# matter-labs/era-zkevm_test_harness

Measured on AMD Instinct MI355X. Metric: base-layer circuits/sec (2^20 rows); full-block synth wall-time 1/8 GPU, higher is better.
Workload: dtype u64 (Goldilocks, p = 2^64 - 2^32 + 1)

## Files before the change

### era_zkevm_test_harness_amd/csrc/poseidon2.cuh

```cuda
#pragma once
#include "gl64.cuh"
#include "../../include/zkw_poseidon2_params.h"

namespace p2 {
using gl::u32;
using gl::u64;

static __constant__ u64 c_rc[P2_TOTAL_ROUNDS * P2_WIDTH] = P2_ROUND_CONSTANTS_INIT;
static __constant__ u32 c_shift[P2_WIDTH] = P2_INTERNAL_DIAG_SHIFTS_INIT;

__host__ __device__ __forceinline__ u64 rc_at(int i) {
#if defined(__HIP_DEVICE_COMPILE__)
    return c_rc[i];
#else
    return P2_ROUND_CONSTANTS[i];
#endif
}
__host__ __device__ __forceinline__ u32 shift_at(int i) {
#if defined(__HIP_DEVICE_COMPILE__)
    return c_shift[i];
#else
    return P2_INTERNAL_DIAG_SHIFTS[i];
#endif
}

struct Wide {
    u64 lo;
    u32 hi;
};
GL_HD Wide wide(u64 x) { Wide r; r.lo = x; r.hi = 0; return r; }
GL_HD Wide wadd(Wide a, Wide b) {
    Wide r;
    r.lo = a.lo + b.lo;
    r.hi = a.hi + b.hi + (r.lo < a.lo ? 1u : 0u);
    return r;
}
GL_HD Wide wshl(Wide a, u32 s) {
    Wide r;
    r.lo = a.lo << s;
    r.hi = (a.hi << s) | (u32)(a.lo >> (64 - s));
    return r;
}
GL_HD u64 wreduce(Wide a) {
    u64 t = ((u64)a.hi << 32) - a.hi;
    u64 r = a.lo + t;
    u64 c = r < t ? gl::EPS : 0;
    return r + c;
}

GL_HD void m4w(const u64 x[4], Wide t[4]) {
    Wide t0 = wadd(wide(x[0]), wide(x[1])), t1 = wadd(wide(x[2]), wide(x[3]));
    Wide t2 = wadd(wshl(wide(x[1]), 1), t1), t3 = wadd(wshl(wide(x[3]), 1), t0);
    Wide t4 = wadd(wshl(t1, 2), t3), t5 = wadd(wshl(t0, 2), t2);
    t[0] = wadd(t3, t5); t[1] = t5; t[2] = wadd(t2, t4); t[3] = t4;
}

#if defined(__HIP_DEVICE_COMPILE__)
__device__ __forceinline__ u64 mad_acc(u32 a, u32 k, u64 acc) {
    u64 r, dead;
    asm("v_mad_u64_u32 %0, %1, %2, %3, %4" : "=v"(r), "=s"(dead) : "v"(a), "s"(k), "v"(acc));
    return r;
}
__device__ __forceinline__ u64 mad_acc1(u32 a, u64 acc) {
    u64 r, dead;
    asm("v_mad_u64_u32 %0, %1, %2, 1, %3" : "=v"(r), "=s"(dead) : "v"(a), "v"(acc));
    return r;
}
__device__ __forceinline__ u64 mad_acc2(u32 a, u64 acc) {
    u64 r, dead;
    asm("v_mad_u64_u32 %0, %1, %2, 2, %3" : "=v"(r), "=s"(dead) : "v"(a), "v"(acc));
    return r;
}
__device__ __forceinline__ u64 wp_reduce(u64 L, u64 H) {
    const u32 l0 = (u32)L, l1 = (u32)(L >> 32), h0 = (u32)H, h1 = (u32)(H >> 32);
    u32 n1, k, f;
    u64 c, c2, dead, r;
    asm("v_add_co_u32_e64 %0, %1, %2, %3" : "=v"(n1), "=s"(c) : "v"(l1), "v"(h0));
    asm("v_addc_co_u32_e64 %0, %1, %2, 0, %3" : "=v"(k), "=s"(dead) : "v"(h1), "s"(c));
    const u64 x = ((u64)n1 << 32) | l0;
    asm("v_mad_u64_u32 %0, %1, %2, -1, %3" : "=v"(r), "=s"(c2) : "v"(k), "v"(x));
    asm("v_cndmask_b32_e64 %0, 0, 1, %1" : "=v"(f) : "s"(c2));
    asm("v_mad_u64_u32 %0, %1, %2, -1, %3" : "=v"(r), "=s"(dead) : "v"(f), "v"(r));
    return r;
}
__device__ __forceinline__ void m4_plane(u32 a0, u32 a1, u32 a2, u32 a3, u64 y[4]) {
    const u64 t0 = mad_acc1(a0, (u64)a1), t1 = mad_acc1(a2, (u64)a3);
    const u64 t2 = mad_acc2(a1, t1), t3 = mad_acc2(a3, t0);
    const u64 t4 = (t1 << 2) + t3, t5 = (t0 << 2) + t2;
    y[0] = t3 + t5; y[1] = t5; y[2] = t2 + t4; y[3] = t4;
}
#endif

GL_HD void external(u64 s[12]) {
#if defined(__HIP_DEVICE_COMPILE__) && !defined(P2_LINEAR_WIDE)
    u64 L[12], H[12];
#pragma unroll
    for (int b = 0; b < 3; b++) {
        m4_plane((u32)s[4 * b], (u32)s[4 * b + 1], (u32)s[4 * b + 2], (u32)s[4 * b + 3], L + 4 * b);
        m4_plane((u32)(s[4 * b] >> 32), (u32)(s[4 * b + 1] >> 32), (u32)(s[4 * b + 2] >> 32), (u32)(s[4 * b + 3] >> 32), H + 4 * b);
    }
#pragma unroll
    for (int i = 0; i < 4; i++) {
        const u64 cl = L[i] + L[4 + i] + L[8 + i], ch = H[i] + H[4 + i] + H[8 + i];
#pragma unroll
        for (int b = 0; b < 3; b++) s[4 * b + i] = wp_reduce(L[4 * b + i] + cl, H[4 * b + i] + ch);
    }
#else
    Wide t[12];
    m4w(s, t); m4w(s + 4, t + 4); m4w(s + 8, t + 8);
#pragma unroll
    for (int i = 0; i < 4; i++) {
        Wide col = wadd(wadd(t[i], t[4 + i]), t[8 + i]);
        s[i] = wreduce(wadd(t[i], col)); s[4 + i] = wreduce(wadd(t[4 + i], col)); s[8 + i] = wreduce(wadd(t[8 + i], col));
    }
#endif
}

GL_HD void internal(u64 s[12]) {
    constexpr u32 SH[12] = P2_INTERNAL_DIAG_SHIFTS_INIT;
#if defined(__HIP_DEVICE_COMPILE__) && !defined(P2_LINEAR_WIDE)
    u64 sl = (u64)(u32)s[0], sh = s[0] >> 32;
#pragma unroll
    for (int i = 1; i < 12; i++) { sl = mad_acc1((u32)s[i], sl); sh = mad_acc1((u32)(s[i] >> 32), sh); }
#pragma unroll
    for (int i = 0; i < 12; i++) {
        const u64 l = SH[i] ? mad_acc((u32)s[i], 1u << SH[i], sl) : mad_acc1((u32)s[i], sl);
        const u64 h = SH[i] ? mad_acc((u32)(s[i] >> 32), 1u << SH[i], sh) : mad_acc1((u32)(s[i] >> 32), sh);
        s[i] = wp_reduce(l, h);
    }
#else
    Wide sum = wide(s[0]);
#pragma unroll
    for (int i = 1; i < 12; i++) sum = wadd(sum, wide(s[i]));
#pragma unroll
    for (int i = 0; i < 12; i++) s[i] = wreduce(wadd(SH[i] ? wshl(wide(s[i]), SH[i]) : wide(s[i]), sum));
#endif
}

#ifndef P2_SBOX_GROUP
#define P2_SBOX_GROUP 3
#endif
template <bool LAT = false>
GL_HD void full_round(u64 s[12], int r) {
#pragma unroll
    for (int i = 0; i < 12; i++) {
        s[i] = LAT ? gl::pow7_lat(gl::add_canon(s[i], rc_at(12 * r + i))) : gl::pow7(gl::add_canon(s[i], rc_at(12 * r + i)));
#if defined(__HIP_DEVICE_COMPILE__)
        if (!LAT && (i + 1) % P2_SBOX_GROUP == 0) __builtin_amdgcn_sched_barrier(0);
#endif
    }
    external(s);
}

template <bool LAT = false>
GL_HD void partial_round(u64 s[12], int r) {
    s[0] = LAT ? gl::pow7_lat(gl::add_canon(s[0], rc_at(12 * r))) : gl::pow7(gl::add_canon(s[0], rc_at(12 * r)));
    internal(s);
}

template <bool LAT = false>
GL_HD void permute(u64 s[12]) {
    external(s);
    int r = 0;
    for (int k = 0; k < P2_HALF_FULL_ROUNDS; k++, r++) full_round<LAT>(s, r);
    for (int k = 0; k < P2_PARTIAL_ROUNDS; k++, r++) partial_round<LAT>(s, r);
    for (int k = 0; k < P2_HALF_FULL_ROUNDS; k++, r++) full_round<LAT>(s, r);
}
GL_HD void permute_lat(u64 s[12]) { permute<true>(s); }

#if defined(__HIPCC__)
template <int CTRL>
__device__ __forceinline__ u32 dpp32(u32 v) {
    return (u32)__builtin_amdgcn_update_dpp((int)0, (int)v, CTRL, 0xF, 0xF, false);
}
template <int CTRL>
__device__ __forceinline__ u64 dpp64(u64 v) {
    u32 lo = dpp32<CTRL>((u32)v), hi = dpp32<CTRL>((u32)(v >> 32));
    return ((u64)hi << 32) | lo;
}
constexpr int QP_ROT1 = 1 | (2 << 2) | (3 << 4) | (0 << 6);
constexpr int QP_ROT2 = 2 | (3 << 2) | (0 << 4) | (1 << 6);
constexpr int QP_ROT3 = 3 | (0 << 2) | (1 << 4) | (2 << 6);
constexpr int QP_SWAP1 = 1 | (0 << 2) | (3 << 4) | (2 << 6);
constexpr int QP_BCAST0 = 0;
constexpr int ROW_ROR4 = 0x124, ROW_ROR8 = 0x128, ROW_ROR12 = 0x12C;

template <int CTRL>
__device__ __forceinline__ Wide wdpp(Wide a) {
    Wide r;
    r.lo = dpp64<CTRL>(a.lo);
    r.hi = dpp32<CTRL>(a.hi);
    return r;
}
__device__ __forceinline__ u64 add_rc_sched(u64 x, u64 c) {
    u32 r0, r1, m;
    asm("v_add_co_u32 %0, vcc, %3, %5\n\t"
        "v_addc_co_u32 %1, vcc, %4, %6, vcc\n\t"
        "v_cndmask_b32 %2, 0, -1, vcc\n\t"
        "v_add_co_u32 %0, vcc, %0, %2\n\t"
        "v_addc_co_u32 %1, vcc, 0, %1, vcc"
        : "=&v"(r0), "=&v"(r1), "=&v"(m)
        : "v"((u32)x), "v"((u32)(x >> 32)), "v"((u32)c), "v"((u32)(c >> 32))
        : "vcc");
    return ((u64)r1 << 32) | r0;
}
#if defined(GL_CHAIN_MUL_COMPILER_FORM)
#define P2_ROW_MUL gl::mul_sched
#else
#define P2_ROW_MUL gl::mul_vcc
#endif
__device__ __forceinline__ u64 pow7_sched(u64 x) {
    const u64 x2 = P2_ROW_MUL(x, x), x3 = P2_ROW_MUL(x2, x), x4 = P2_ROW_MUL(x2, x2);
    return P2_ROW_MUL(x3, x4);
}

struct Coop {
    u64 rc_full[2 * P2_HALF_FULL_ROUNDS];
    u32 ka, kb, kd;
    u32 shift;
    u32 rsh, hi_mask;
    bool active;
    bool first;
    bool second;

    __device__ __forceinline__ void init(int g) {
        active = g < 12;
        first = g == 0;
        second = g == 1;
#pragma unroll
        for (int k = 0; k < 2 * P2_HALF_FULL_ROUNDS; k++) {
            int round = k < P2_HALF_FULL_ROUNDS ? k : k + P2_PARTIAL_ROUNDS;
            rc_full[k] = active ? c_rc[12 * round + g] : 0;
        }
        bool even = (g & 1) == 0;
        ka = even ? 5u : 6u;
        kb = even ? 7u : 1u;
        kd = even ? 3u : 4u;
        shift = active ? c_shift[g] : 0;
        rsh = (32u - shift) & 31u;
        hi_mask = shift ? 0xffffffffu : 0u;
    }

    __device__ __forceinline__ u64 external(u64 x) const {
        u64 a = x, b = dpp64<QP_ROT1>(x), c = dpp64<QP_ROT2>(x), d = dpp64<QP_ROT3>(x);
        u64 L = (a & gl::EPS) * ka + (b & gl::EPS) * kb + (c & gl::EPS) + (d & gl::EPS) * kd;
        u64 H = (a >> 32) * ka + (b >> 32) * kb + (c >> 32) + (d >> 32) * kd;
        u32 r0, r1, t0, t1, t2, u0, u1, u2, e0, e1, e2;
        asm volatile(
            "v_add_co_u32 %3, vcc, %11, %13\n\t"
            "v_addc_co_u32 %4, vcc, 0, %14, vcc\n\t"
            "s_nop 0\n\t"
            "v_add_co_u32_dpp %5, vcc, %12, %12 row_ror:8 row_mask:0xf bank_mask:0xf\n\t"
            "v_addc_co_u32_dpp %6, vcc, %3, %3, vcc row_ror:8 row_mask:0xf bank_mask:0xf\n\t"
            "v_addc_co_u32_dpp %7, vcc, %4, %4, vcc row_ror:8 row_mask:0xf bank_mask:0xf\n\t"
            "v_add_co_u32_dpp %5, vcc, %5, %5 row_ror:4 row_mask:0xf bank_mask:0xf\n\t"
            "v_addc_co_u32_dpp %6, vcc, %6, %6, vcc row_ror:4 row_mask:0xf bank_mask:0xf\n\t"
            "v_addc_co_u32_dpp %7, vcc, %7, %7, vcc row_ror:4 row_mask:0xf bank_mask:0xf\n\t"
            "v_add_co_u32 %0, vcc, %12, %5\n\t"
            "v_addc_co_u32 %1, vcc, %3, %6, vcc\n\t"
            "v_addc_co_u32 %2, vcc, %4, %7, vcc\n\t"
            "v_sub_co_u32 %8, vcc, 0, %2\n\t"
            "v_subbrev_co_u32 %9, vcc, 0, %2, vcc\n\t"
            "v_add_co_u32 %0, vcc, %0, %8\n\t"
            "v_addc_co_u32 %1, vcc, %1, %9, vcc\n\t"
            "v_cndmask_b32 %10, 0, -1, vcc\n\t"
            "v_add_co_u32 %0, vcc, %0, %10\n\t"
            "v_addc_co_u32 %1, vcc, 0, %1, vcc"
            : "=&v"(r0), "=&v"(r1), "=&v"(t0), "=&v"(t1), "=&v"(t2), "=&v"(u0), "=&v"(u1), "=&v"(u2), "=&v"(e0), "=&v"(e1), "=&v"(e2)
            : "v"((u32)(L >> 32)), "v"((u32)L), "v"((u32)H), "v"((u32)(H >> 32))
            : "vcc");
        const u64 y = ((u64)r1 << 32) | r0;
        return active ? y : 0;
    }

    __device__ __forceinline__ u64 internal(u64 x) const {
        const u32 x0 = (u32)x, x1 = (u32)(x >> 32);
        u32 s0, s1, s2;
        const u32 zero = 0;
        asm volatile(
            "s_nop 1\n\t"
            "v_add_co_u32_dpp %0, vcc, %3, %3 row_ror:8 row_mask:0xf bank_mask:0xf\n\t"
            "v_addc_co_u32_dpp %1, vcc, %4, %4, vcc row_ror:8 row_mask:0xf bank_mask:0xf\n\t"
            "v_addc_co_u32 %2, vcc, 0, %5, vcc\n\t"
            "v_add_co_u32_dpp %0, vcc, %0, %0 row_ror:4 row_mask:0xf bank_mask:0xf\n\t"
            "v_addc_co_u32_dpp %1, vcc, %1, %1, vcc row_ror:4 row_mask:0xf bank_mask:0xf\n\t"
            "v_addc_co_u32_dpp %2, vcc, %2, %2, vcc row_ror:4 row_mask:0xf bank_mask:0xf\n\t"
            "v_add_co_u32_dpp %0, vcc, %0, %0 quad_perm:[2,3,0,1] row_mask:0xf bank_mask:0xf\n\t"
            "v_addc_co_u32_dpp %1, vcc, %1, %1, vcc quad_perm:[2,3,0,1] row_mask:0xf bank_mask:0xf\n\t"
            "v_addc_co_u32_dpp %2, vcc, %2, %2, vcc quad_perm:[2,3,0,1] row_mask:0xf bank_mask:0xf\n\t"
            "v_add_co_u32_dpp %0, vcc, %0, %0 quad_perm:[1,0,3,2] row_mask:0xf bank_mask:0xf\n\t"
            "v_addc_co_u32_dpp %1, vcc, %1, %1, vcc quad_perm:[1,0,3,2] row_mask:0xf bank_mask:0xf\n\t"
            "v_addc_co_u32_dpp %2, vcc, %2, %2, vcc quad_perm:[1,0,3,2] row_mask:0xf bank_mask:0xf"
            : "=&v"(s0), "=&v"(s1), "=&v"(s2)
            : "v"(x0), "v"(x1), "v"(zero)
            : "vcc");
        const u64 mlo = x << shift;
        const u32 m2 = (x1 >> rsh) & hi_mask;
        u32 r0, r1;
        u32 t0, t1, t2, t3;
        asm volatile(
            "v_add_co_u32 %0, vcc, %6, %9\n\t"
            "v_addc_co_u32 %1, vcc, %7, %10, vcc\n\t"
            "v_addc_co_u32 %2, vcc, %8, %11, vcc\n\t"
            "v_sub_co_u32 %3, vcc, 0, %2\n\t"
            "v_subbrev_co_u32 %4, vcc, 0, %2, vcc\n\t"
            "v_add_co_u32 %0, vcc, %0, %3\n\t"
            "v_addc_co_u32 %1, vcc, %1, %4, vcc\n\t"
            "v_cndmask_b32 %5, 0, -1, vcc\n\t"
            "v_add_co_u32 %0, vcc, %0, %5\n\t"
            "v_addc_co_u32 %1, vcc, 0, %1, vcc"
            : "=&v"(r0), "=&v"(r1), "=&v"(t0), "=&v"(t1), "=&v"(t2), "=&v"(t3)
            : "v"((u32)mlo), "v"((u32)(mlo >> 32)), "v"(m2), "v"(s0), "v"(s1), "v"(s2)
            : "vcc");
        const u64 y = ((u64)r1 << 32) | r0;
        return active ? y : 0;
    }

    __device__ __forceinline__ u64 permute(u64 x) const {
        x = external(x);
#pragma unroll
        for (int k = 0; k < P2_HALF_FULL_ROUNDS; k++) x = external(pow7_sched(add_rc_sched(x, rc_full[k])));
        for (int k = 0; k < P2_PARTIAL_ROUNDS; k++) {
            u64 rc = c_rc[12 * (P2_HALF_FULL_ROUNDS + k)];
            u64 sx = pow7_pair(add_rc_sched(x, rc));
            x = internal(first ? sx : x);
        }
#pragma unroll
        for (int k = 0; k < P2_HALF_FULL_ROUNDS; k++)
            x = external(pow7_sched(add_rc_sched(x, rc_full[P2_HALF_FULL_ROUNDS + k])));
        return x;
    }

    __device__ __forceinline__ u64 pow7_pair(u64 t) const {
        const u64 t0 = dpp64<QP_BCAST0>(t);
        const u64 x2 = P2_ROW_MUL(t0, t0);
        const u64 b = second ? x2 : t0;
        const u64 y = P2_ROW_MUL(x2, b);
        return P2_ROW_MUL(y, dpp64<QP_SWAP1>(y));
    }
};

template <class Put>
__device__ __forceinline__ u64 coop_flattened(const Coop& co, u64 x, u32 g, Put&& put) {
    if (co.active) put(g, gl::canon(x));
    x = co.external(x);
#pragma unroll
    for (int k = 0; k < P2_HALF_FULL_ROUNDS; k++) {
        x = co.external(pow7_sched(add_rc_sched(x, co.rc_full[k])));
        if (co.active) put(12 * (k + 1) + g, gl::canon(x));
    }
    for (int k = 0; k < P2_PARTIAL_ROUNDS; k++) {
        const u64 rc = c_rc[12 * (P2_HALF_FULL_ROUNDS + k)];
        const u64 sx = co.pow7_pair(add_rc_sched(x, rc));
        if (co.first) put(12 * (P2_HALF_FULL_ROUNDS + 1) + k, gl::canon(sx));
        x = co.internal(co.first ? sx : x);
    }
#pragma unroll
    for (int k = 0; k < P2_HALF_FULL_ROUNDS; k++) {
        x = co.external(pow7_sched(add_rc_sched(x, co.rc_full[P2_HALF_FULL_ROUNDS + k])));
        if (co.active) put(12 * (P2_HALF_FULL_ROUNDS + 1) + P2_PARTIAL_ROUNDS + 12 * k + g, gl::canon(x));
    }
    return gl::canon(x);
}


__device__ __forceinline__ u64 q4_mul(u64 a, u64 b) {
#if defined(GL_CHAIN_MUL_COMPILER_FORM)
    return gl::mul_lat(a, b);
#else
    return gl::mul_vcc(a, b);
#endif
}
__device__ __forceinline__ u64 q4_pow7(u64 x) {
    const u64 x2 = q4_mul(x, x), x3 = q4_mul(x2, x), x4 = q4_mul(x2, x2);
    return q4_mul(x3, x4);
}
template <int CTRL>
__device__ __forceinline__ u32 qdpp32(u32 v) {
    return (u32)__builtin_amdgcn_update_dpp((int)0, (int)v, CTRL, 0xF, 0xF, true);
}
template <int CTRL>
__device__ __forceinline__ u64 qdpp64(u64 v) {
    return ((u64)qdpp32<CTRL>((u32)(v >> 32)) << 32) | qdpp32<CTRL>((u32)v);
}

struct Coop4 {
    u64 rc_full[2 * P2_HALF_FULL_ROUNDS][3];
    u32 ka, kb, kd;
    u32 pw[3];
    bool first;
    bool second;

    __device__ __forceinline__ void init(int j) {
        first = j == 0;
        second = j == 1;
#pragma unroll
        for (int k = 0; k < 2 * P2_HALF_FULL_ROUNDS; k++) {
            int round = k < P2_HALF_FULL_ROUNDS ? k : k + P2_PARTIAL_ROUNDS;
#pragma unroll
            for (int c = 0; c < 3; c++) rc_full[k][c] = c_rc[12 * round + 4 * c + j];
        }
        bool even = (j & 1) == 0;
        ka = even ? 5u : 6u;
        kb = even ? 7u : 1u;
        kd = even ? 3u : 4u;
#pragma unroll
        for (int c = 0; c < 3; c++) pw[c] = 1u << c_shift[4 * c + j];
    }

#if defined(__HIP_DEVICE_COMPILE__)
    static __device__ __forceinline__ u64 mad_v(u32 a, u32 k, u64 acc) {
        u64 r, dead;
        asm("v_mad_u64_u32 %0, %1, %2, %3, %4" : "=v"(r), "=s"(dead) : "v"(a), "v"(k), "v"(acc));
        return r;
    }
    template <bool SC = false>
    static __device__ __forceinline__ u64 add_rc(u64 x, u32 c0, u32 c1);
#endif

    __device__ __forceinline__ u64 m4_plane(u32 a) const {
        const u32 b = qdpp32<QP_ROT1>(a), c = qdpp32<QP_ROT2>(a), d = qdpp32<QP_ROT3>(a);
#if defined(__HIP_DEVICE_COMPILE__)
        return mad_v(d, kd, mad_v(b, kb, mad_v(a, ka, (u64)c)));
#else
        return (u64)a * ka + (u64)b * kb + c + (u64)d * kd;
#endif
    }

    __device__ __forceinline__ void external(u64 x[3]) const {
#if defined(__HIP_DEVICE_COMPILE__)
        u64 L[3], H[3];
#pragma unroll
        for (int c = 0; c < 3; c++) { L[c] = m4_plane((u32)x[c]); H[c] = m4_plane((u32)(x[c] >> 32)); }
        const u64 cl = L[0] + L[1] + L[2], ch = H[0] + H[1] + H[2];
#pragma unroll
        for (int c = 0; c < 3; c++) x[c] = wp_reduce(L[c] + cl, H[c] + ch);
#endif
    }

    __device__ __forceinline__ void internal(u64 x[3]) const {
#if defined(__HIP_DEVICE_COMPILE__)
        const u64 pl = mad_acc1((u32)x[0], mad_acc1((u32)x[1], (u64)(u32)x[2]));
        const u64 ph = mad_acc1((u32)(x[0] >> 32), mad_acc1((u32)(x[1] >> 32), x[2] >> 32));
        u32 l0, l1, h0, h1;
        asm volatile(
            "s_nop 1\n\t"
            "v_add_co_u32_dpp %0, vcc, %4, %4 quad_perm:[2,3,0,1] row_mask:0xf bank_mask:0xf\n\t"
            "v_addc_co_u32_dpp %1, vcc, %5, %5, vcc quad_perm:[2,3,0,1] row_mask:0xf bank_mask:0xf\n\t"
            "v_add_co_u32_dpp %2, vcc, %6, %6 quad_perm:[2,3,0,1] row_mask:0xf bank_mask:0xf\n\t"
            "v_addc_co_u32_dpp %3, vcc, %7, %7, vcc quad_perm:[2,3,0,1] row_mask:0xf bank_mask:0xf\n\t"
            "v_add_co_u32_dpp %0, vcc, %0, %0 quad_perm:[1,0,3,2] row_mask:0xf bank_mask:0xf\n\t"
            "v_addc_co_u32_dpp %1, vcc, %1, %1, vcc quad_perm:[1,0,3,2] row_mask:0xf bank_mask:0xf\n\t"
            "v_add_co_u32_dpp %2, vcc, %2, %2 quad_perm:[1,0,3,2] row_mask:0xf bank_mask:0xf\n\t"
            "v_addc_co_u32_dpp %3, vcc, %3, %3, vcc quad_perm:[1,0,3,2] row_mask:0xf bank_mask:0xf"
            : "=&v"(l0), "=&v"(l1), "=&v"(h0), "=&v"(h1)
            : "v"((u32)pl), "v"((u32)(pl >> 32)), "v"((u32)ph), "v"((u32)(ph >> 32))
            : "vcc");
        const u64 sl = ((u64)l1 << 32) | l0, sh = ((u64)h1 << 32) | h0;
#pragma unroll
        for (int c = 0; c < 3; c++) x[c] = wp_reduce(mad_v((u32)x[c], pw[c], sl), mad_v((u32)(x[c] >> 32), pw[c], sh));
#endif
    }

    __device__ __forceinline__ void permute(u64 x[3]) const {
#if defined(__HIP_DEVICE_COMPILE__)
        constexpr u64 RC[P2_TOTAL_ROUNDS * P2_WIDTH] = P2_ROUND_CONSTANTS_INIT;
        external(x);
#pragma unroll
// ... 124 lines not shown
```

### era_zkevm_test_harness_amd/csrc/ram_circuit_kernels.cuh

```cuda
#pragma once
#include "../../include/zkw_ram_circuit_spec.h"
#include "../../include/zkw_decommit_sorter_circuit_spec.h"
#include "../../include/zkw_events_sorter_circuit_spec.h"
#include "ram_kernels.cuh"
#include "public_input_kernels.cuh"
#include "closed_form_kernels.cuh"

namespace zkw {

struct SynthJob {
    const zkw_ram_instance* inst;
    const zkw_mem_query* sorted_q;
    const zkw_mem_query* unsorted_q;
    const u64* unsorted_caps;
    const u64* sorted_caps;
    const u64* u_mark;
    const u64* s_mark;
    const u64* challenges;
    const u64* gp_ckpt;
    u64* trace;
    u32* hist;
    const u32* nd_tiles;
    const u64* public_input;
    const zkw_ram_instance* first_inst;
    u32 tail_clean;
};

constexpr int RC_INLINE_JOBS = 32;
struct SynthJobsRef {
    const SynthJob* p;
    __device__ __forceinline__ const SynthJob& operator[](unsigned k) const { return p[k]; }
};
struct SynthJobsInline {
    SynthJob j[RC_INLINE_JOBS];
    __device__ __forceinline__ const SynthJob& operator[](unsigned k) const { return j[k]; }
};
static_assert(sizeof(SynthJobsInline) <= 3968, "the inline job table and the scalar arguments share the 4 KB of kernel arguments");

constexpr int ROW_SLOTS[RC_NUM_ROW_TYPES] = RC_ROW_NUM_SLOTS_INIT;
constexpr int ROW_LOOKUPS[RC_NUM_ROW_TYPES] = RC_ROW_NUM_LOOKUPS_INIT;
static_assert(ROW_SLOTS[RC_ROW_PU] == 133 && ROW_SLOTS[RC_ROW_PS] == 130, "Poseidon2 rows: 130 gate variables (+3 spare in PU)");
static_assert(ROW_LOOKUPS[RC_ROW_PU] == 12 && ROW_LOOKUPS[RC_ROW_PS] == 12 && ROW_LOOKUPS[RC_ROW_A] == 12 &&
              ROW_LOOKUPS[RC_ROW_B] == 12 && ROW_LOOKUPS[RC_ROW_C] == 8 && ROW_LOOKUPS[RC_ROW_D] == 0,
              "lookup cells per cycle (56) are hard-wired in the fill kernels");
constexpr int LOOKUPS_PER_CYCLE = 56;

__device__ __forceinline__ u64 inv_or_zero(u64 x) { return gl::canon(x) ? gl::inv(x) : 0; }

struct RegsIn {
    const u64* uh;
    const u64* sh;
    u32 len;
};
__device__ __forceinline__ RegsIn regs_in(const zkw_ram_instance* in) {
    RegsIn r;
    const bool start = in->start_flag != 0;
    r.uh = start ? in->unsorted_queue_initial_state.head : in->hidden_fsm_input.current_unsorted_queue_state.head;
    r.sh = start ? in->sorted_queue_initial_state.head : in->hidden_fsm_input.current_sorted_queue_state.head;
    r.len = start ? in->unsorted_queue_initial_state.length : in->hidden_fsm_input.current_unsorted_queue_state.length;
    return r;
}

#define TR(col, row) trace[(size_t)(col) * n_rows + (row)]

__device__ __forceinline__ void zero_gap_row(u64* trace, size_t n_rows, size_t row) {
    for (int col = 0; col < RC_G + RC_L; col++) TR(col, row) = 0;
}
__device__ __forceinline__ void zero_gap_row_n(u64* trace, size_t n_rows, size_t row, int n_cols) {
    for (int col = 0; col < n_cols; col++) TR(col, row) = 0;
}

__device__ __forceinline__ void hist_bytes(u32* sh_hist, u32 x) {
    atomicAdd(&sh_hist[x & 0xFF], 1u);
    atomicAdd(&sh_hist[(x >> 8) & 0xFF], 1u);
    atomicAdd(&sh_hist[(x >> 16) & 0xFF], 1u);
    atomicAdd(&sh_hist[x >> 24], 1u);
}
__device__ __forceinline__ void put_bytes(u64* trace, size_t n_rows, size_t row, int col0, u32 x) {
    TR(col0, row) = x & 0xFF;
    TR(col0 + 1, row) = (x >> 8) & 0xFF;
    TR(col0 + 2, row) = (x >> 16) & 0xFF;
    TR(col0 + 3, row) = x >> 24;
}
__device__ __forceinline__ void hist_flush(u32* sh_hist, u32* g_hist) {
    __syncthreads();
    for (int t = threadIdx.x; t < 256; t += blockDim.x)
        if (sh_hist[t]) atomicAdd(&g_hist[t], sh_hist[t]);
}

__device__ __forceinline__ void fill_flattened_poseidon(u64* trace, size_t n_rows, size_t row, u64 s[12]) {
    int pos = 0;
#pragma unroll
    for (int k = 0; k < 12; k++) TR(pos++, row) = gl::canon(s[k]);
    p2::external(s);
    int r = 0;
    for (int k = 0; k < P2_HALF_FULL_ROUNDS; k++, r++) {
        p2::full_round(s, r);
#pragma unroll
        for (int j = 0; j < 12; j++) TR(pos + j, row) = gl::canon(s[j]);
        pos += 12;
    }
    for (int k = 0; k < P2_PARTIAL_ROUNDS; k++, r++) {
        s[0] = gl::pow7(gl::add_canon(s[0], p2::rc_at(12 * r)));
        TR(pos++, row) = gl::canon(s[0]);
        p2::internal(s);
    }
    for (int k = 0; k < P2_HALF_FULL_ROUNDS; k++, r++) {
        p2::full_round(s, r);
#pragma unroll
        for (int j = 0; j < 12; j++) TR(pos + j, row) = gl::canon(s[j]);
        pos += 12;
    }
}

struct CycleCtx {
    bool can_pop;
    zkw_mem_query q, pq;
    u64 es[8];
    u64 p_val[5];
    u32 p_ptr;
};

__device__ __forceinline__ void load_query(const zkw_mem_query* src, zkw_mem_query& dst) {
    const uint4* s = reinterpret_cast<const uint4*>(src);
    uint4* d = reinterpret_cast<uint4*>(&dst);
    d[0] = s[0]; d[1] = s[1]; d[2] = s[2];
}

__device__ __forceinline__ void cycle_ctx(const SynthJob& job, u32 i, CycleCtx& c) {
    const zkw_ram_instance* in = job.inst;
    const size_t first = in->first_item, m = in->num_items;
    c.can_pop = i < m;
    memset(&c.q, 0, sizeof c.q);
    memset(&c.pq, 0, sizeof c.pq);
#pragma unroll
    for (int k = 0; k < 8; k++) c.es[k] = 0;
    if (c.can_pop) {
        load_query(job.sorted_q + first + i, c.q);
        encode_mem_query(c.q, c.es);
    }
    if (i == 0) {
        const zkw_ram_fsm& f = in->hidden_fsm_input;
        c.pq.timestamp = f.previous_sorting_key[0]; c.pq.index = f.previous_sorting_key[1]; c.pq.page = f.previous_sorting_key[2];
        for (int k = 0; k < 8; k++) c.pq.value[k] = f.previous_value[k];
        c.pq.value_is_pointer = f.previous_is_ptr ? 1 : 0;
    } else if (i - 1 < m) {
        load_query(job.sorted_q + first + i - 1, c.pq);
    }
    u64 pe[8];
    encode_mem_query(c.pq, pe);
#pragma unroll
    for (int k = 0; k < 5; k++) c.p_val[k] = pe[3 + k];
    c.p_ptr = c.pq.value_is_pointer ? 1 : 0;
}

__device__ __forceinline__ void acc_before_pair(u64 fl, u64 fr, u64 ckpt_l, u64 ckpt_r, int lane, u64& pl, u64& pr) {
#pragma unroll
    for (int d = 1; d < 64; d <<= 1) {
        const u64 ol = __shfl_up(fl, d, 64), orr = __shfl_up(fr, d, 64);
        if (lane >= d) { fl = gl::mul(fl, ol); fr = gl::mul(fr, orr); }
        __builtin_amdgcn_sched_barrier(0);
    }
    const u64 el = __shfl_up(fl, 1, 64), er = __shfl_up(fr, 1, 64);
    pl = lane == 0 ? ckpt_l : gl::canon(gl::mul(ckpt_l, el));
    pr = lane == 0 ? ckpt_r : gl::canon(gl::mul(ckpt_r, er));
    __builtin_amdgcn_sched_barrier(0);
}

__device__ __forceinline__ void fill_row_A(const SynthJob& job, u32 i, u32 capacity, size_t n_rows, const zkw_mem_query& q,
                                           const u64 eu[8], const u64 es[8], u32* sh_hist) {
    u64* trace = job.trace;
    const size_t row = (size_t)RC_ROW_A * RC_REGION_STRIDE(capacity) + i;
    const bool live = i < capacity;
    const bool can_pop = live && i < job.inst->num_items;
    const int lane = threadIdx.x & 63;
    const u64* ckpt = job.gp_ckpt + 4 * (size_t)((u32)__builtin_amdgcn_readfirstlane((int)i) >> 6);
    if (live) {
#pragma unroll
        for (int k = 0; k < 8; k++) { TR(RC_A_eu0 + k, row) = eu[k]; TR(RC_A_ts + k, row) = es[k]; }
    }
    for (int r = 0; r < 2; r++) {
        const u64* ch = job.challenges + 9 * r;
        u64 lc = ch[8], rc = ch[8];
#pragma unroll
        for (int k = 0; k < 8; k++) {
            lc = gl::add(lc, gl::mul(eu[k], ch[k]));
            rc = gl::add(rc, gl::mul(es[k], ch[k]));
            __builtin_amdgcn_sched_barrier(0);
        }
        u64 pl, pr;
        acc_before_pair(can_pop ? lc : 1, can_pop ? rc : 1, ckpt[r], ckpt[2 + r], lane, pl, pr);
        if (live) {
            const u64 nl = gl::canon(gl::mul(pl, lc)), nr = gl::canon(gl::mul(pr, rc));
            const int o = r * (RC_A_lc1 - RC_A_lc0);
#pragma unroll
            for (int k = 1; k < 9; k++) TR(RC_A_G_c0_1 + (k - 1) + r * (RC_A_G_c1_1 - RC_A_G_c0_1), row) = ch[k];
            __builtin_amdgcn_sched_barrier(0);
            TR(RC_A_lc0 + o, row) = gl::canon(lc); TR(RC_A_P_lhs0 + o, row) = pl; TR(RC_A_nl0 + o, row) = nl;
            TR(RC_A_lhs0 + o, row) = can_pop ? nl : pl;
            TR(RC_A_rc0 + o, row) = gl::canon(rc); TR(RC_A_P_rhs0 + o, row) = pr; TR(RC_A_nr0 + o, row) = nr;
            TR(RC_A_rhs0 + o, row) = can_pop ? nr : pr;
        }
        __builtin_amdgcn_sched_barrier(0);
    }
    if (live) {
        const u64 rw = q.rw_flag ? 1 : 0, ptr = q.value_is_pointer ? 1 : 0;
        TR(RC_A_rw, row) = rw; TR(RC_A_ptr, row) = ptr; TR(RC_A_idx, row) = q.index;
        TR(RC_A_v2, row) = q.value[2]; TR(RC_A_v3, row) = q.value[3]; TR(RC_A_v0, row) = q.value[0];
        TR(RC_A_v5_b3c, row) = q.value[5] >> 24; TR(RC_A_can_pop, row) = can_pop ? 1 : 0;
        put_bytes(trace, n_rows, row, RC_A_v2_b0, q.value[2]);
        put_bytes(trace, n_rows, row, RC_A_v3_b0, q.value[3]);
        put_bytes(trace, n_rows, row, RC_A_v5_b0, q.value[5]);
        hist_bytes(sh_hist, q.value[2]); hist_bytes(sh_hist, q.value[3]); hist_bytes(sh_hist, q.value[5]);
        constexpr int NA = ROW_SLOTS[RC_ROW_A];
        if (!job.tail_clean) {
            for (int col = NA; col < RC_G; col++) TR(col, row) = 0;
            for (int col = RC_G + 12; col < RC_G + RC_L; col++) TR(col, row) = 0;
        }
    } else if (i < RC_REGION_STRIDE(capacity)) {
        if (!job.tail_clean) zero_gap_row(trace, n_rows, row);
    }
}

__device__ __forceinline__ void fill_row_B(const SynthJob& job, u32 i, u32 capacity, size_t n_rows, const zkw_mem_query& q,
                                           const u64 es[8], u32* sh_hist) {
    u64* trace = job.trace;
    const size_t row = (size_t)RC_ROW_B * RC_REGION_STRIDE(capacity) + i;
    if (i < capacity) {
        const zkw_ram_instance* in = job.inst;
        u32 p_ts = 0;
        if (i == 0) p_ts = in->hidden_fsm_input.previous_sorting_key[0];
        else if (i - 1 < in->num_items) p_ts = job.sorted_q[in->first_item + i - 1].timestamp;
        put_bytes(trace, n_rows, row, RC_B_v6_b0, q.value[6]);
        put_bytes(trace, n_rows, row, RC_B_v7_b0, q.value[7]);
        TR(RC_B_es4, row) = es[4]; TR(RC_B_v1, row) = q.value[1]; TR(RC_B_v5_b3c, row) = q.value[5] >> 24;
        TR(RC_B_es5, row) = es[5]; TR(RC_B_v2, row) = q.value[2];
        TR(RC_B_es6, row) = es[6]; TR(RC_B_v3, row) = q.value[3];
        const u32 d0 = q.timestamp - p_ts;
        TR(RC_B_d0, row) = d0; put_bytes(trace, n_rows, row, RC_B_d0_b0, d0);
        TR(RC_B_bw0, row) = q.timestamp < p_ts ? 1 : 0;
        TR(RC_B_ts, row) = q.timestamp; TR(RC_B_P_ts, row) = p_ts;
        hist_bytes(sh_hist, q.value[6]); hist_bytes(sh_hist, q.value[7]); hist_bytes(sh_hist, d0);
        constexpr int NB = ROW_SLOTS[RC_ROW_B];
        if (!job.tail_clean) {
            for (int col = NB; col < RC_G; col++) TR(col, row) = 0;
            for (int col = RC_G + 12; col < RC_G + RC_L; col++) TR(col, row) = 0;
        }
    } else if (i < RC_REGION_STRIDE(capacity)) {
        if (!job.tail_clean) zero_gap_row(trace, n_rows, row);
    }
}

template <int SIDE>
__device__ __forceinline__ void ram_poseidon_prologue(const SynthJob& job, u32 i, u32 capacity, size_t n_rows, size_t row, bool can_pop,
                                                      u64 s[12], u32* sh_hist) {
    u64* trace = job.trace;
    const size_t first = job.inst->first_item;
    zkw_mem_query q;
    memset(&q, 0, sizeof q);
    if (can_pop) {
        load_query(job.sorted_q + first + i, q);
        if (SIDE == 0) encode_raw_query(load_raw_query(job.unsorted_q + first + i), s); else encode_mem_query(q, s);
    }
    if (SIDE == 0) {
        u64 es[8];
        encode_mem_query(q, es);
        fill_row_A(job, i, capacity, n_rows, q, s, es, sh_hist);
    } else {
        fill_row_B(job, i, capacity, n_rows, q, s, sh_hist);
    }
    if (i < capacity) {
        if (SIDE == 0) {
            TR(RC_PU_idx, row) = q.index; TR(RC_PU_v0, row) = q.value[0]; TR(RC_PU_v1, row) = q.value[1];
            put_bytes(trace, n_rows, row, RC_PU_idx_b0, q.index);
            put_bytes(trace, n_rows, row, RC_PU_v0_b0, q.value[0]);
            put_bytes(trace, n_rows, row, RC_PU_v1_b0, q.value[1]);
            hist_bytes(sh_hist, q.index); hist_bytes(sh_hist, q.value[0]); hist_bytes(sh_hist, q.value[1]);
        } else {
            if (!job.tail_clean) for (int c = 130; c < RC_G; c++) TR(c, row) = 0;
            put_bytes(trace, n_rows, row, RC_PS_ts_b0, q.timestamp);
            put_bytes(trace, n_rows, row, RC_PS_page_b0, q.page);
            put_bytes(trace, n_rows, row, RC_PS_v4_b0, q.value[4]);
            hist_bytes(sh_hist, q.timestamp); hist_bytes(sh_hist, q.page); hist_bytes(sh_hist, q.value[4]);
        }
        if (!job.tail_clean) for (int c = RC_G + 12; c < RC_G + RC_L; c++) TR(c, row) = 0;
    }
}

template <class J>
static __device__ __forceinline__ void k_ram_fill_poseidon(const VB& vb, const J& jobs, u32 capacity, size_t n_rows) {
    __shared__ u32 sh_hist[256];
    for (int t = threadIdx.x; t < 256; t += blockDim.x) sh_hist[t] = 0;
    __syncthreads();
    const SynthJob job = jobs[vb.y];
    const u32 side = vb.z;
    const u32 i = vb.x * blockDim.x + threadIdx.x;
    u64* trace = job.trace;
    const zkw_ram_instance* in = job.inst;
    const size_t first = in->first_item, m = in->num_items;
    const bool can_pop = i < capacity && i < m;
    const size_t row = (size_t)(side == 0 ? RC_ROW_PU : RC_ROW_PS) * RC_REGION_STRIDE(capacity) + i;
    u64 s[12];
#pragma unroll
    for (int k = 0; k < 8; k++) s[k] = 0;
    if (side == 0) ram_poseidon_prologue<0>(job, i, capacity, n_rows, row, can_pop, s, sh_hist);
    else ram_poseidon_prologue<1>(job, i, capacity, n_rows, row, can_pop, s, sh_hist);
    if (i < capacity) {
        __builtin_amdgcn_sched_barrier(0);
        const RegsIn ri = regs_in(in);
        const u64* caps = side == 0 ? job.unsorted_caps : job.sorted_caps;
        const u64* prev_cap = i == 0 ? (side == 0 ? ri.uh : ri.sh) + 8 : caps + 4 * (first + (i - 1 < m ? i - 1 : m - 1));
#pragma unroll
        for (int k = 0; k < 4; k++) s[8 + k] = prev_cap[k];
        fill_flattened_poseidon(trace, n_rows, row, s);
    } else if (i < RC_REGION_STRIDE(capacity)) {
        if (!job.tail_clean) zero_gap_row(trace, n_rows, row);
    }
    hist_flush(sh_hist, job.hist);
}

__device__ __forceinline__ bool nd_flag(bool can_pop, const zkw_mem_query& q) {
    return can_pop && q.timestamp == 0 && q.page == RC_HEAP_PAGE && q.rw_flag && !q.value_is_pointer;
}

template <class J>
static __device__ __forceinline__ void k_ram_fill_C(const VB& vb, const J& jobs, u32 capacity, size_t n_rows) {
    __shared__ u32 sh_hist[256];
    __shared__ u32 sh_wave[4];
    sh_hist[threadIdx.x] = 0;
    __syncthreads();
    const SynthJob job = jobs[vb.y];
    const u32 i = vb.x * blockDim.x + threadIdx.x;
    const bool live = i < capacity;
    CycleCtx c;
    c.can_pop = false;
    bool nd = false;
    if (live) {
        cycle_ctx(job, i, c);
        nd = nd_flag(c.can_pop, c.q);
    }
    const unsigned long long bal = __ballot(nd);
    const int lane = threadIdx.x & 63, wave = threadIdx.x >> 6;
    if (lane == 0) sh_wave[wave] = __popcll(bal);
    __syncthreads();
    u32 before = __popcll(bal & ((1ull << lane) - 1));
    for (int w = 0; w < wave; w++) before += sh_wave[w];
    if (live) {
        u64* trace = job.trace;
        const zkw_ram_instance* in = job.inst;
        const size_t row = (size_t)RC_ROW_C * RC_REGION_STRIDE(capacity) + i;
        const u64 rw = c.q.rw_flag ? 1 : 0, ptr = c.q.value_is_pointer ? 1 : 0;
        const u64 bw0 = c.q.timestamp < c.pq.timestamp ? 1 : 0;
        const u64 t1 = (u64)c.pq.index + bw0, bw1 = (u64)c.q.index < t1 ? 1 : 0;
        const u32 d1 = (u32)((u64)c.q.index - t1);
        const u64 t2 = (u64)c.pq.page + bw1, bw2 = (u64)c.q.page < t2 ? 1 : 0;
        const u32 d2 = (u32)((u64)c.q.page - t2);
        TR(RC_C_d1, row) = d1; put_bytes(trace, n_rows, row, RC_C_d1_b0, d1);
        TR(RC_C_d2, row) = d2; put_bytes(trace, n_rows, row, RC_C_d2_b0, d2);
        hist_bytes(sh_hist, d1); hist_bytes(sh_hist, d2);
        TR(RC_C_bw1, row) = bw1; TR(RC_C_bw2, row) = bw2; TR(RC_C_bw0, row) = bw0;
        TR(RC_C_idx, row) = c.q.index; TR(RC_C_P_idx, row) = c.pq.index;
        TR(RC_C_page, row) = c.q.page; TR(RC_C_P_page, row) = c.pq.page;
        TR(RC_C_can_pop, row) = c.can_pop ? 1 : 0;
        u64 x[14];
        x[0] = gl::canon(gl::sub(c.q.index, c.pq.index));
        x[1] = gl::canon(gl::sub(c.q.page, c.pq.page));
        const u64 val[5] = {c.es[3], c.es[4], c.es[5], c.es[6], c.es[7]};
#pragma unroll
        for (int k = 0; k < 5; k++) { x[2 + k] = gl::canon(gl::sub(val[k], c.p_val[k])); x[7 + k] = val[k]; }
        x[12] = c.q.timestamp;
        x[13] = gl::canon(gl::sub(c.q.page, RC_HEAP_PAGE));
        u64 pre[14], acc = 1;
#pragma unroll
        for (int k = 0; k < 14; k++) { pre[k] = acc; acc = gl::mul(acc, x[k] ? x[k] : 1); }
        u64 inv = gl::inv(acc), w[14];
#pragma unroll
        for (int k = 13; k >= 0; k--) {
            w[k] = x[k] ? gl::canon(gl::mul(inv, pre[k])) : 0;
            inv = gl::mul(inv, x[k] ? x[k] : 1);
        }
        const u64 z_idx = x[0] == 0, z_page = x[1] == 0, same = z_idx & z_page;
        TR(RC_C_w_idx, row) = w[0]; TR(RC_C_z_idx, row) = z_idx;
        TR(RC_C_w_page, row) = w[1]; TR(RC_C_z_page, row) = z_page; TR(RC_C_same, row) = same;
        const int C_VAL[5] = {RC_C_es3, RC_C_es4, RC_C_es5, RC_C_es6, RC_C_v4};
        const int C_PVAL[5] = {RC_C_P_es3, RC_C_P_es4, RC_C_P_es5, RC_C_P_es6, RC_C_P_v4};
        const int C_WEQ[5] = {RC_C_w_eq0, RC_C_w_eq1, RC_C_w_eq2, RC_C_w_eq3, RC_C_w_eq4};
        const int C_ZEQ[5] = {RC_C_z_eq0, RC_C_z_eq1, RC_C_z_eq2, RC_C_z_eq3, RC_C_z_eq4};
        const int C_WZ[5] = {RC_C_w_z0, RC_C_w_z1, RC_C_w_z2, RC_C_w_z3, RC_C_w_z4};
        const int C_ZZ[5] = {RC_C_z_z0, RC_C_z_z1, RC_C_z_z2, RC_C_z_z3, RC_C_z_z4};
        u64 zeq[5], zz[5];
#pragma unroll
        for (int k = 0; k < 5; k++) {
            zeq[k] = x[2 + k] == 0; zz[k] = x[7 + k] == 0;
            TR(C_VAL[k], row) = val[k]; TR(C_PVAL[k], row) = c.p_val[k];
            TR(C_WEQ[k], row) = w[2 + k]; TR(C_ZEQ[k], row) = zeq[k];
            TR(C_WZ[k], row) = w[7 + k]; TR(C_ZZ[k], row) = zz[k];
        }
        const u64 peq = ptr == c.p_ptr, eq_a = zeq[0] & zeq[1] & zeq[2], value_equal = eq_a & zeq[3] & zeq[4] & peq;
        const u64 zz_a = zz[0] & zz[1] & zz[2], all_zero = zz_a & zz[3] & zz[4] & (1 - ptr);
        TR(RC_C_ptr, row) = ptr; TR(RC_C_P_ptr, row) = c.p_ptr; TR(RC_C_peq, row) = peq;
        TR(RC_C_eq_a, row) = eq_a; TR(RC_C_value_equal, row) = value_equal;
        TR(RC_C_zz_a, row) = zz_a; TR(RC_C_all_zero, row) = all_zero; TR(RC_C_rw, row) = rw;
        TR(RC_C_ts, row) = c.q.timestamp; TR(RC_C_w_ts, row) = w[12]; TR(RC_C_z_ts, row) = x[12] == 0;
        TR(RC_C_w_heap, row) = w[13]; TR(RC_C_z_heap, row) = x[13] == 0; TR(RC_C_nd, row) = nd ? 1 : 0;
        const u64 p_cnt = (u64)in->hidden_fsm_input.num_nondeterministic_writes + job.nd_tiles[vb.x] + before;
        TR(RC_C_P_cnt, row) = p_cnt; TR(RC_C_cnt, row) = p_cnt + (nd ? 1 : 0);
        constexpr int NC = ROW_SLOTS[RC_ROW_C];
        if (!job.tail_clean) {
            for (int col = NC; col < RC_G; col++) TR(col, row) = 0;
// ... 393 lines not shown
```

Baseline: 3429.

## Fuse Poseidon2 partial rounds in pairs with shared 32-bit MAD accumulation

Replaces the per-round partial-round loop with a pairwise fused version. Two consecutive internal-matrix applications share their row-sum and diagonal accumulations through v_mad_u64_u32 on 32-bit limbs, and the next round constant is folded into the accumulator, so one reduction per lane covers two rounds. The aim is to cut the repeated sum and reduce work in the partial rounds, which dominate permutation cost. Both permute and the trace-filling path now use it. The cost is inline asm tied to the diagonal-shift structure and more complex carry handling, which is a correctness risk if limb sums overflow.

```diff
diff --git a/era_zkevm_test_harness_amd/csrc/poseidon2.cuh b/era_zkevm_test_harness_amd/csrc/poseidon2.cuh
--- a/era_zkevm_test_harness_amd/csrc/poseidon2.cuh
+++ b/era_zkevm_test_harness_amd/csrc/poseidon2.cuh
@@ -158,12 +158,94 @@
     internal(s);
 }
 
+static_assert(P2_PARTIAL_ROUNDS % 2 == 0, "the partial rounds are walked in pairs");
+#if defined(__HIP_DEVICE_COMPILE__) && !defined(P2_LINEAR_WIDE) && !defined(P2_PARTIAL_SINGLE)
+#define P2_PAIR_FUSED 1
+__device__ __forceinline__ u64 mad_mul(u32 a, u32 k) {
+    u64 r, dead;
+    asm("v_mad_u64_u32 %0, %1, %2, %3, 0" : "=v"(r), "=s"(dead) : "v"(a), "s"(k));
+    return r;
+}
+__device__ __forceinline__ u64 mad_sacc1(u32 c, u64 acc) {
+    u64 r, dead;
+    asm("v_mad_u64_u32 %0, %1, %2, 1, %3" : "=v"(r), "=s"(dead) : "s"(c), "v"(acc));
+    return r;
+}
+template <bool NEXT>
+__device__ __forceinline__ void partial_pair_fused(u64 s[12], u64 cB, u64 cn, u64& sa, u64& sb) {
+    constexpr u32 SH[12] = P2_INTERNAL_DIAG_SHIFTS_INIT;
+    u64 Pl = (u64)(u32)s[1], Ph = s[1] >> 32;
+    u64 Rl = mad_mul((u32)s[1], (1u << SH[1]) + 11u), Rh = mad_mul((u32)(s[1] >> 32), (1u << SH[1]) + 11u);
+#pragma unroll
+    for (int i = 2; i < 12; i++) {
+        Pl = mad_acc1((u32)s[i], Pl); Ph = mad_acc1((u32)(s[i] >> 32), Ph);
+        Rl = mad_acc((u32)s[i], (1u << SH[i]) + 11u, Rl); Rh = mad_acc((u32)(s[i] >> 32), (1u << SH[i]) + 11u, Rh);
+    }
+    const u64 s0 = gl::pow7(s[0]);
+    sa = s0;
+    const u64 Sl = mad_acc1((u32)s0, Pl), Sh = mad_acc1((u32)(s0 >> 32), Ph);
+    const u64 y0 = wp_reduce(mad_sacc1((u32)cB, mad_acc((u32)s0, 1u << SH[0], Sl)), mad_sacc1((u32)(cB >> 32), mad_acc((u32)(s0 >> 32), 1u << SH[0], Sh)));
+    const u64 Sr = wp_reduce(Sl, Sh);
+    Rl = mad_acc((u32)s0, 11u, Rl); Rh = mad_acc((u32)(s0 >> 32), 11u, Rh);
+    const u64 t0 = gl::pow7(y0);
+    sb = t0;
+    const u64 Tl = mad_acc1((u32)t0, Rl), Th = mad_acc1((u32)(t0 >> 32), Rh);
+    u64 zl = mad_acc((u32)t0, 1u << SH[0], Tl), zh = mad_acc((u32)(t0 >> 32), 1u << SH[0], Th);
+    if (NEXT) { zl = mad_sacc1((u32)cn, zl); zh = mad_sacc1((u32)(cn >> 32), zh); }
+    s[0] = wp_reduce(zl, zh);
+#pragma unroll
+    for (int i = 1; i < 12; i++) {
+        const u64 l = SH[i] ? mad_acc((u32)Sr, 1u << SH[i], mad_acc((u32)s[i], 1u << 2 * SH[i], Tl)) : mad_acc1((u32)Sr, mad_acc1((u32)s[i], Tl));
+        const u64 h = SH[i] ? mad_acc((u32)(Sr >> 32), 1u << SH[i], mad_acc((u32)(s[i] >> 32), 1u << 2 * SH[i], Th))
+                            : mad_acc1((u32)(Sr >> 32), mad_acc1((u32)(s[i] >> 32), Th));
+        s[i] = wp_reduce(l, h);
+    }
+}
+#endif
+
+GL_HD void partial_pair(u64 s[12], int r, u64& sbox_a, u64& sbox_b) {
+#if defined(P2_PAIR_FUSED)
+    s[0] = gl::add_canon(s[0], rc_at(12 * r));
+    partial_pair_fused<false>(s, rc_at(12 * (r + 1)), 0, sbox_a, sbox_b);
+#else
+    sbox_a = s[0] = gl::pow7(gl::add_canon(s[0], rc_at(12 * r)));
+    internal(s);
+    sbox_b = s[0] = gl::pow7(gl::add_canon(s[0], rc_at(12 * (r + 1))));
+    internal(s);
+#endif
+}
+
+template <class Put>
+GL_HD void partial_rounds(u64 s[12], int r, Put&& put) {
+#if defined(P2_PAIR_FUSED)
+    s[0] = gl::add_canon(s[0], rc_at(12 * r));
+    for (int k = 0; k < P2_PARTIAL_ROUNDS; k += 2) {
+        const u64 cn = rc_at(12 * (r + k + 2)) & (k + 2 < P2_PARTIAL_ROUNDS ? ~0ull : 0ull);
+        u64 a, b;
+        partial_pair_fused<true>(s, rc_at(12 * (r + k + 1)), cn, a, b);
+        put(k, a);
+        put(k + 1, b);
+    }
+#else
+    for (int k = 0; k < P2_PARTIAL_ROUNDS; k++) {
+        s[0] = gl::pow7(gl::add_canon(s[0], rc_at(12 * (r + k))));
+        put(k, s[0]);
+        internal(s);
+    }
+#endif
+}
+
 template <bool LAT = false>
 GL_HD void permute(u64 s[12]) {
     external(s);
     int r = 0;
     for (int k = 0; k < P2_HALF_FULL_ROUNDS; k++, r++) full_round<LAT>(s, r);
-    for (int k = 0; k < P2_PARTIAL_ROUNDS; k++, r++) partial_round<LAT>(s, r);
+    if constexpr (LAT) {
+        for (int k = 0; k < P2_PARTIAL_ROUNDS; k++, r++) partial_round<LAT>(s, r);
+    } else {
+        partial_rounds(s, r, [](int, u64) {});
+        r += P2_PARTIAL_ROUNDS;
+    }
     for (int k = 0; k < P2_HALF_FULL_ROUNDS; k++, r++) full_round<LAT>(s, r);
 }
 GL_HD void permute_lat(u64 s[12]) { permute<true>(s); }
diff --git a/era_zkevm_test_harness_amd/csrc/ram_circuit_kernels.cuh b/era_zkevm_test_harness_amd/csrc/ram_circuit_kernels.cuh
--- a/era_zkevm_test_harness_amd/csrc/ram_circuit_kernels.cuh
+++ b/era_zkevm_test_harness_amd/csrc/ram_circuit_kernels.cuh
@@ -100,11 +100,9 @@
         for (int j = 0; j < 12; j++) TR(pos + j, row) = gl::canon(s[j]);
         pos += 12;
     }
-    for (int k = 0; k < P2_PARTIAL_ROUNDS; k++, r++) {
-        s[0] = gl::pow7(gl::add_canon(s[0], p2::rc_at(12 * r)));
-        TR(pos++, row) = gl::canon(s[0]);
-        p2::internal(s);
-    }
+    p2::partial_rounds(s, r, [&](int k, u64 sbox) { TR(pos + k, row) = gl::canon(sbox); });
+    pos += P2_PARTIAL_ROUNDS;
+    r += P2_PARTIAL_ROUNDS;
     for (int k = 0; k < P2_HALF_FULL_ROUNDS; k++, r++) {
         p2::full_round(s, r);
 #pragma unroll
```

Result: no change. 3459, median of 6 (+0.9%).
